# bcsefercik/markerless-robot-camera-calibration

Measured on AMD Instinct MI355X. Metric: point-cloud frames/sec at 200k pts/frame, higher is better.
Workload: dtype f32

## Files before the change

### markerless-robot-camera-calibration_amd/_lib.py

```python
import ctypes
import os
from ctypes import c_char_p, c_double, c_float, c_int, c_int64, c_size_t, c_void_p

import torch

_HERE = os.path.dirname(os.path.abspath(__file__))
ABI_VERSION = 4
LIB_PATH = os.environ.get("SVHIP_LIB") or os.path.join(_HERE, "libsvhip.so")

SV_ACT_NONE, SV_ACT_RELU, SV_ACT_LEAKY_RELU = 0, 1, 2
SV_POOL_MAX, SV_POOL_AVG = 0, 1
SV_REDUCE_MEAN, SV_REDUCE_FIRST = 0, 1
SV_TILE_ROWS = 128
SV_ERR_UNSUPPORTED = -5
SV_PN_MAX_LAYERS = 4
SV_PN_MAX_SCALES = 4
SV_BQ_MAX_RADII = 4
SV_GROUP_SSG, SV_GROUP_MSG = 0, 1
SV_LOSS_POSE, SV_LOSS_SHAPE_MATCH, SV_LOSS_POSE_MATCH, SV_LOSS_KP_POSE_MATCH = 0, 1, 2, 3
SV_AUG_STRIDE, SV_AUG_ELASTIC0, SV_AUG_ELASTIC1 = 40, 0, 7
SV_AUG_E_ON, SV_AUG_E_OFFSET, SV_AUG_E_BX, SV_AUG_E_BY, SV_AUG_E_BZ, SV_AUG_E_GRAN, SV_AUG_E_MAG = range(7)
SV_AUG_NOISE_ON, SV_AUG_NOISE_SIGMA, SV_AUG_NOISE_CLIP, SV_AUG_TRANSFORM_ON, SV_AUG_ROT, SV_AUG_TRANSLATION = 14, 15, 16, 17, 18, 27
SV_AUG_FLIP_SIGN, SV_AUG_GRAVITY_ON, SV_AUG_GRAVITY_ANGLE, SV_AUG_GRAVITY_COS, SV_AUG_GRAVITY_SIN = 30, 31, 32, 33, 34
SV_ORIGIN_NONE, SV_ORIGIN_CENTER, SV_ORIGIN_BASE = 0, 1, 2
SV_COORD_BIAS = 1 << 17
SV_COORD_BITS = 18
SV_MAX_BATCH = 1024
SV_FRAME_MAX_LEVELS, SV_FRAME_MAX_CUTS, SV_FRAME_RECORD = 8, 4, 16
SV_FRAME_K3, SV_FRAME_DOWN, SV_FRAME_UP, SV_FRAME_SPLIT = 1, 2, 4, 8
SV_FIELD_F32, SV_FIELD_F64 = 7, 8
SV_UNPACK_BIGENDIAN, SV_UNPACK_KEEP_NONFINITE = 1, 2
SV_DEPTH_U16, SV_DEPTH_F32 = 4, 7
SV_RGBD_ALIGNED, SV_RGBD_NEAREST, SV_RGBD_BGR = 1, 2, 4
SV_FRAME_REC_HASH, SV_FRAME_REC_K3, SV_FRAME_REC_DOWN, SV_FRAME_REC_UP, SV_FRAME_REC_SPLIT = 1, 2, 3, 4, 5


class SvHipError(RuntimeError):
    pass


_P = c_void_p
SIGNATURES = {
    "sv_last_error": (c_char_p, []),
    "sv_abi_version": (c_int, []),
    "sv_voxelize_workspace_bytes": (c_size_t, [c_int64]),
    "sv_voxelize": (c_int, [_P, c_int, c_int64, _P, c_size_t, _P, _P, _P, _P, _P, _P, _P]),
    "sv_voxel_reduce": (c_int, [_P, c_int, _P, _P, c_int64, c_int, _P, _P]),
    "sv_hash_build": (c_int, [_P, c_int64, _P, _P, c_int64, _P]),
    "sv_stride_map_workspace_bytes": (c_size_t, [c_int64]),
    "sv_stride_map": (c_int, [_P, c_int64, c_int, _P, c_size_t, _P, _P, _P, _P, _P, _P]),
    "sv_kernel_map_k3": (c_int, [_P, c_int64, c_int, c_int, _P, _P, c_int64, _P, c_int64, _P, _P]),
    "sv_kernel_map_down": (c_int, [_P, _P, c_int64, c_int, c_int64, _P, c_int64, _P, _P]),
    "sv_kernel_map_up": (c_int, [_P, _P, c_int64, c_int, _P, c_int64, _P, _P]),
    "sv_plan_workspace_bytes": (c_size_t, [c_int64]),
# ... 110 lines not shown
_lib = None


def load():
    global _lib
    if _lib is not None:
        return _lib
    if not os.path.exists(LIB_PATH):
        raise SvHipError(
            f"{LIB_PATH} not found: build it with `python -c 'import __graft_entry__ as g; g.build()'` "
            "(or `make -C markerless-robot-camera-calibration_amd/csrc`). There is no CPU fallback."
        )
    lib = ctypes.CDLL(LIB_PATH)
    lib.sv_abi_version.restype = c_int
    if lib.sv_abi_version() != ABI_VERSION:
        raise SvHipError(f"{LIB_PATH} has C-ABI version {lib.sv_abi_version()}, this package binds version {ABI_VERSION}: "
                         "rebuild it (`python -c 'import __graft_entry__ as g; g.build()'`)")
    for name, (res, args) in SIGNATURES.items():
        fn = getattr(lib, name)
        fn.restype = res
        fn.argtypes = args
    _lib = lib
    return lib


def _check(rc, name):
    if rc != 0:
        msg = _lib.sv_last_error().decode("utf-8", "replace")
        raise SvHipError(f"{name} failed with status {rc}: {msg}")


def ptr(t):
    if t is None:
        return None
    return c_void_p(t.data_ptr())


def stream_ptr():
    return c_void_p(torch.cuda.current_stream().cuda_stream)


def call(name, *args):
    lib = load()
    rc = getattr(lib, name)(*args)
    _check(rc, name)


def conv_last_instance():
    raw = load().sv_conv_last_instance().decode()
    name, _, flags = raw.partition("|")
    return name, {k: int(v) for k, v in (kv.split("=") for kv in flags.split(",") if kv)}


class conv_dispatch:

    def __init__(self, want_scale, tail_fraction=-1.0):
        self.args = (c_double(want_scale), c_double(tail_fraction))

    def __enter__(self):
        call("sv_conv_set_dispatch", *self.args)

    def __exit__(self, *exc):
        call("sv_conv_set_dispatch", c_double(-1.0), c_double(-1.0))


def require_cuda(t, what="tensor"):
    if not t.is_cuda:
        raise SvHipError(f"{what} must live on the GPU (got {t.device}); the HIP path has no CPU fallback")
    return t
```

### markerless-robot-camera-calibration_amd/csrc/sv_conv.hip

```cpp
#include <stdarg.h>
#include <stdio.h>
#include <stdlib.h>
#include <vector>

#include "sv_conv_params.h"

namespace sv {

static thread_local char g_last_instance[128] = "";
static thread_local double g_want_scale_override = -1.0;
static thread_local double g_tail_override = -1.0;
void note_instance(const char* fmt, ...) {
  va_list ap;
  va_start(ap, fmt);
  vsnprintf(g_last_instance, sizeof(g_last_instance), fmt, ap);
  va_end(ap);
}
#ifndef SV_CONV_WANT_SCALE_DEFAULT
#define SV_CONV_WANT_SCALE_DEFAULT 0.3
#endif
#ifndef SV_CONV_TAIL_DEFAULT
#define SV_CONV_TAIL_DEFAULT 0.15
#endif
constexpr int chunk_for(int tm, int waves_n) {
// ... 752 lines not shown
  SV_CHECK_ARG(in_ld >= Cin && out_ld >= Cout, "row strides too small");
  SV_CHECK_ARG(act >= SV_ACT_NONE && act <= SV_ACT_LEAKY_RELU, "bad activation");
  if (V_out == 0) return SV_OK;
  SV_CHECK_ARG(in && W && out, "null pointer");
  SV_CHECK_ARG(V_in >= 1, "V_in = rows of `in` (every index of the plan is below it)");
  const bool has_plan = perm || nbr_s || submask;
  SV_CHECK_ARG(!has_plan || (perm && nbr_s && submask), "perm, nbr_s and submask must be given together");
  SV_CHECK_ARG(has_plan || K == 1, "K > 1 needs a plan");
  SV_CHECK_ARG(!residual || res_ld >= Cout, "residual stride too small");
  ConvParams p;
  p.in = in; p.in_ld = in_ld; p.Cin = Cin; p.W = W; p.K = K; p.Cout = Cout;
  p.perm = perm; p.nbr_s = nbr_s; p.submask = submask; p.tile_order = tile_order; p.V_out = V_out; p.Vpad = Vpad;
  p.scale = scale; p.shift = shift; p.residual = residual; p.res_ld = res_ld;
  p.acc_init = acc_init; p.acc_ld = acc_ld;
  p.act = act; p.slope = slope; p.out = out; p.out_ld = out_ld;
  p.vec_a = (in_ld % 4 == 0) && (Cin % 4 == 0) && (((uintptr_t)in & 15) == 0);
  const uint64_t in_bytes = ((uint64_t)(V_in - 1) * (uint64_t)in_ld + (uint64_t)Cin) * 4u;
  const uint64_t w_bytes = (uint64_t)K * (uint64_t)Cin * (uint64_t)Cout * 4u;
  const uint64_t out_bytes = ((uint64_t)(V_out - 1) * (uint64_t)out_ld + (uint64_t)Cout) * 4u;
  const uint64_t res_bytes = residual ? ((uint64_t)(V_out - 1) * (uint64_t)res_ld + (uint64_t)Cout) * 4u : 0u;
  const uint64_t acc_bytes = acc_init ? ((uint64_t)(V_out - 1) * (uint64_t)acc_ld + (uint64_t)Cout) * 4u : 0u;
  p.buf_ok = in_bytes < BUF_LIMIT && w_bytes < BUF_LIMIT && out_bytes < BUF_LIMIT && res_bytes < BUF_LIMIT &&
             acc_bytes < BUF_LIMIT && (((uintptr_t)perm & 15) == 0);
  p.acc_bytes = p.buf_ok ? (uint32_t)acc_bytes : 0u;
  if (!p.buf_ok && !has_plan && K == 1 && w_bytes < BUF_LIMIT) {
    int64_t ld_max = in_ld > out_ld ? in_ld : out_ld;
    if (residual && res_ld > ld_max) ld_max = res_ld;
    const int64_t rows = (int64_t)((BUF_LIMIT - 4096u) / ((uint64_t)ld_max * 4u)) / PLAN_TILE * PLAN_TILE;
    if (rows >= PLAN_TILE && rows < V_out) {
      for (int64_t r0 = 0; r0 < V_out; r0 += rows) {
        const int64_t n = V_out - r0 < rows ? V_out - r0 : rows;
        const int rc = sv_conv_fwd_acc(in + r0 * in_ld, n, in_ld, Cin, W, K, Cout, nullptr, nullptr, nullptr, nullptr, n,
                                       (n + PLAN_TILE - 1) / PLAN_TILE * PLAN_TILE, acc_init ? acc_init + r0 * acc_ld : nullptr,
                                       acc_ld, scale, shift, residual ? residual + r0 * res_ld : nullptr, res_ld, act, slope,
                                       out + r0 * out_ld, out_ld, stream_);
        if (rc != SV_OK) return rc;
      }
      return SV_OK;
    }
  }
  p.in_bytes = p.buf_ok ? (uint32_t)in_bytes : 0u;
  p.w_bytes = p.buf_ok ? (uint32_t)w_bytes : 0u;
  p.out_bytes = p.buf_ok ? (uint32_t)out_bytes : 0u;
  p.res_bytes = p.buf_ok ? (uint32_t)res_bytes : 0u;
  p.ntiles = 0;
  p.ny = 0;
  p.trace = nullptr;
  p.main_blocks = 0;
  p.main_tiles128 = 0;
  if (has_plan && K > 1 && K <= 27 && Cin == 3 && Cout == 32 && !acc_init) {
    if (p.buf_ok) return launch_conv_first_mfma(p, stream);
    return launch_conv_first_layer(p, stream);
  }
  if (has_plan && K > 1 && K <= 32 && Cin == 32 && Cout == 32 && p.vec_a && p.buf_ok && !acc_init)
    return launch_conv_thin(p, stream, sv::g_want_scale_override >= 1.0);
  if (!has_plan && K == 1 && Cout <= 4 && p.vec_a && Cin >= 64 && !acc_init) return launch_linear_narrow(p, stream);
  return select_and_launch(p, stream);
}
```

### markerless-robot-camera-calibration_amd/csrc/sv_conv_params.h

```cpp
#pragma once
#include <type_traits>

#include "sv_common.h"

namespace sv {

typedef float f32x4 __attribute__((ext_vector_type(4)));

struct ConvParams {
  const float* in;
  int64_t in_ld;
  int Cin;
  const float* W;
  int K;
  int Cout;
  const int32_t* perm;
  const int32_t* nbr_s;
  const uint32_t* submask;
  const int32_t* tile_order;
  int64_t V_out;
  int64_t Vpad;
  const float* scale;
  const float* shift;
  const float* residual;
  int64_t res_ld;
  const float* acc_init;
  int64_t acc_ld;
  uint32_t acc_bytes;
  int act;
  float slope;
  float* out;
  int64_t out_ld;
  int vec_a;
  uint32_t in_bytes, w_bytes, out_bytes, res_bytes;
  int buf_ok;
  int ntiles;
  int ny;
  unsigned long long* trace;
  int main_blocks;
  int main_tiles128;
};

constexpr int PLAN_TILE = SV_TILE_ROWS;
void note_instance(const char* fmt, ...);
int launch_conv_first_mfma(const ConvParams& p, hipStream_t stream);
int launch_conv_first_layer(const ConvParams& p, hipStream_t stream);
int launch_conv_thin(const ConvParams& p, hipStream_t stream, bool alone);
int launch_linear_narrow(const ConvParams& p, hipStream_t stream);

constexpr uint32_t BUF_ABSENT = 0x80000000u;
constexpr uint32_t BUF_LIMIT = 0x7fff0000u;
typedef int i32x4_t __attribute__((ext_vector_type(4)));
typedef int i32x3_t __attribute__((ext_vector_type(3)));
typedef int i32x2_t __attribute__((ext_vector_type(2)));
template <int N>
__device__ __forceinline__ auto buffer_load_floats(__amdgpu_buffer_rsrc_t rsrc, uint32_t voffset, uint32_t soffset) {
  typedef float vec_t __attribute__((ext_vector_type(N)));
  if constexpr (N == 1) {
    vec_t r;
    r[0] = __builtin_bit_cast(float, __builtin_amdgcn_raw_buffer_load_b32(rsrc, voffset, soffset, 0));
    return r;
  } else if constexpr (N == 2) {
    return __builtin_bit_cast(vec_t, __builtin_amdgcn_raw_buffer_load_b64(rsrc, voffset, soffset, 0));
  } else if constexpr (N == 3) {
    return __builtin_bit_cast(vec_t, __builtin_amdgcn_raw_buffer_load_b96(rsrc, voffset, soffset, 0));
  } else {
    static_assert(N == 4, "1..4 floats per load");
    return __builtin_bit_cast(vec_t, __builtin_amdgcn_raw_buffer_load_b128(rsrc, voffset, soffset, 0));
  }
}

template <int MR>
__device__ __forceinline__ void load_perm_rows(const ConvParams& p, const int64_t rows0, const int lq, int (&o)[MR][4]) {
#pragma unroll
  for (int s = 0; s < MR; ++s) {
    const int64_t r = rows0 + s * 16 + lq * 4;
    if (p.perm) {
      const int4 o4 = *(const int4*)(p.perm + r);
      o[s][0] = o4.x;
      o[s][1] = o4.y;
      o[s][2] = o4.z;
      o[s][3] = o4.w;
    } else {
#pragma unroll
      for (int reg = 0; reg < 4; ++reg) o[s][reg] = (r + reg < p.V_out) ? (int)(r + reg) : -1;
    }
  }
}

template <int MR, int NT, bool PRELOADED = false>
__device__ __forceinline__ void epilogue_buffered(const ConvParams& p, const f32x4 (&acc)[MR][NT], const int64_t rows0,
                                                  const int lq, const int col0, const int (*o_pre)[4] = nullptr) {
  typedef float yvec_t __attribute__((ext_vector_type(NT)));
  const __amdgpu_buffer_rsrc_t rsrc_out = __builtin_amdgcn_make_buffer_rsrc((void*)p.out, 0, (int)p.out_bytes, 0x00020000);
  const __amdgpu_buffer_rsrc_t rsrc_res =
      __builtin_amdgcn_make_buffer_rsrc((void*)p.residual, 0, p.residual ? (int)p.res_bytes : 0, 0x00020000);
  int o[MR][4];
// ... 66 lines not shown
```

### markerless-robot-camera-calibration_amd/csrc/sv_conv_special.hip

```cpp
#include <stdio.h>
#include <stdlib.h>
#include <algorithm>
#include <vector>

#include "sv_conv_params.h"

namespace sv {

constexpr int NARROW_ROWS = 64;
template <int C>
__global__ __launch_bounds__(256) void linear_narrow_kernel(ConvParams p) {
  constexpr int ROWS = NARROW_ROWS, COLS = 32, SW = COLS + 1, LPT = ROWS / 32;
  __shared__ float tile[2][ROWS * SW];
  const int tid = threadIdx.x;
  const int64_t row0 = (int64_t)blockIdx.x * ROWS;
  const int Cin = p.Cin;
  const int lr = tid >> 3, lc = (tid & 7) * 4;
  float4 ra[LPT];
  auto load = [&](int c0) {
#pragma unroll
    for (int i = 0; i < LPT; ++i) {
      const int64_t r = row0 + lr + 32 * i;
      const int c = c0 + lc;
      const bool ok = r < p.V_out && c < Cin;
      const float4 v = *(const float4*)(p.in + (ok ? r * p.in_ld + c : 0));
      ra[i] = ok ? v : make_float4(0.f, 0.f, 0.f, 0.f);
    }
  };
  auto store = [&](float* dst) {
#pragma unroll
    for (int i = 0; i < LPT; ++i) {
      float* d = dst + (lr + 32 * i) * SW + lc;
      d[0] = ra[i].x;
      d[1] = ra[i].y;
      d[2] = ra[i].z;
      d[3] = ra[i].w;
    }
  };
  float acc[C];
#pragma unroll
  for (int j = 0; j < C; ++j) acc[j] = 0.0f;
  load(0);
  store(tile[0]);
  __syncthreads();
  int buf = 0;
  for (int c0 = 0; c0 < Cin; c0 += COLS) {
    const bool more = c0 + COLS < Cin;
    if (more) load(c0 + COLS);
    if (tid < ROWS) {
      const float* x = tile[buf] + tid * SW;
      const float* w = p.W + (int64_t)c0 * p.Cout;
      const int nc = min(COLS, Cin - c0);
#pragma unroll 8
      for (int c = 0; c < nc; ++c) {
// ... 359 lines not shown
    SV_HIP(hipGetDeviceProperties(&prop, dev));
    n_cu = prop.multiProcessorCount > 0 ? prop.multiProcessorCount : 256;
    SV_HIP(hipFuncSetAttribute((const void*)conv_thin_lds_kernel<32, 32, D, WAVES>, hipFuncAttributeMaxDynamicSharedMemorySize,
                               (int)(((size_t)27 * 32 * 32 + (size_t)WAVES * (32 * 16)) * sizeof(float))));
    attr_set = true;
  }
  const int n_sub = (int)(p.Vpad / 16);
  const int grid = n_sub < n_cu ? n_sub : n_cu;
  static const bool trace = getenv("SV_THIN_TRACE") != nullptr;
  ConvParams q = p;
  q.trace = nullptr;
  if (trace) {
    SV_HIP(hipMalloc((void**)&q.trace, (size_t)grid * WAVES * 12 * sizeof(unsigned long long)));
    SV_HIP(hipMemsetAsync(q.trace, 0, (size_t)grid * WAVES * 12 * sizeof(unsigned long long), stream));
  }
  hipLaunchKernelGGL((conv_thin_lds_kernel<32, 32, D, WAVES>), dim3((unsigned)grid), dim3(WAVES * 64), lds, stream, q, n_sub);
  note_instance("conv_thin_lds_kernel<32, 32>|fast=1,ring=0,full=1");
  SV_LAUNCH_CHECK();
  if (trace) {
    std::vector<unsigned long long> h((size_t)grid * WAVES * 12);
    SV_HIP(hipStreamSynchronize(stream));
    SV_HIP(hipMemcpy(h.data(), q.trace, h.size() * sizeof(unsigned long long), hipMemcpyDeviceToHost));
    SV_HIP(hipFree(q.trace));
    std::vector<double> stage, table, loop, store, life, per_off, it01, it12, pre;
    for (size_t w = 0; w < (size_t)grid * WAVES; ++w) {
      const unsigned long long* o = &h[w * 12];
      if (!o[0]) continue;
      if (o[8] && o[9] && o[10]) {
        pre.push_back((double)(o[8] - o[2]));
        it01.push_back((double)(o[9] - o[8]));
        it12.push_back((double)(o[10] - o[9]));
      }
      stage.push_back((double)(o[1] - o[0]));
      life.push_back((double)(o[5] - o[0]));
      if (o[6]) {
        table.push_back((double)(o[2] - o[1]));
        loop.push_back((double)(o[3] - o[2]));
        store.push_back((double)(o[4] - o[3]));
        if (o[7]) per_off.push_back((double)(o[3] - o[2]) / (double)o[7]);
      }
    }
    auto med = [](std::vector<double>& v) {
      if (v.empty()) return 0.0;
      std::sort(v.begin(), v.end());
      return v[v.size() / 2];
    };
    fprintf(stderr, "[thin trace] K=%d n_sub=%d grid=%d | median cycles: weights staged %.0f, first tile: table %.0f, loop %.0f "
            "(%.0f per offset; table staged -> loop %.0f, first 4 offsets %.0f, next 4 %.0f), store %.0f, wave life %.0f\n", p.K, n_sub,
            grid, med(stage), med(table), med(loop), med(per_off), med(pre), med(it01), med(it12), med(store), med(life));
  }
  return SV_OK;
}

int launch_conv_thin(const ConvParams& p, hipStream_t stream, bool alone) {
  if (alone && p.K <= 27 && (((uintptr_t)p.W) & 15) == 0) return launch_conv_thin_lds(p, stream);
  hipLaunchKernelGGL((conv_thin_kernel<32, 32, 1, 4>), dim3((unsigned)(p.Vpad / 64)), dim3(256), 0, stream, p);
  note_instance("conv_thin_kernel<32, 32>|fast=1,ring=0,full=1");
  SV_LAUNCH_CHECK();
  return SV_OK;
}

template <int CIN, int COUT, int SPLIT>
__global__ __launch_bounds__(256) void conv_first_layer_kernel(ConvParams p) {
  constexpr int CT = COUT / SPLIT;
  constexpr int KMAX = 27;
  const int tid = threadIdx.x;
  const int K = p.K;
  const int j0 = (int)blockIdx.y * CT;
  const float* __restrict__ w_s = p.W + j0;
  const int64_t r = (int64_t)blockIdx.x * 256 + tid;
  const bool in_range = r < p.Vpad;
  const int64_t o = in_range ? (int64_t)p.perm[r] : -1;
  float acc[CT];
#pragma unroll
  for (int j = 0; j < CT; ++j) acc[j] = 0.0f;
  int n[KMAX];
#pragma unroll
  for (int k = 0; k < KMAX; ++k) n[k] = (o >= 0 && k < K) ? p.nbr_s[(int64_t)k * p.Vpad + r] : -1;
  constexpr int G = 9;
#pragma unroll
  for (int k0 = 0; k0 < KMAX; k0 += G) {
    float x[G][CIN];
#pragma unroll
    for (int g = 0; g < G; ++g) {
      const float* src = p.in + (n[k0 + g] >= 0 ? (int64_t)n[k0 + g] * p.in_ld : 0);
#pragma unroll
      for (int c = 0; c < CIN; ++c) x[g][c] = src[c];
    }
#pragma unroll
    for (int g = 0; g < G; ++g) {
      const bool has = n[k0 + g] >= 0;
      if (__ballot(has) == 0ull) continue;
      const float* w = w_s + (k0 + g) * CIN * COUT;
      if (has) {
#pragma unroll
        for (int c = 0; c < CIN; ++c) {
#pragma unroll
          for (int j = 0; j < CT; ++j) acc[j] = __builtin_fmaf(x[g][c], w[c * COUT + j], acc[j]);
        }
      }
    }
  }
  if (o < 0) return;
  float* dst = p.out + o * p.out_ld + j0;
#pragma unroll
  for (int j = 0; j < CT; ++j) {
    float v = acc[j];
    if (p.scale)
// ... 51 lines not shown
```

### markerless-robot-camera-calibration_amd/nn.py

```python
import math
from ctypes import c_float, c_int, c_int64, c_size_t

import numpy as np
import torch
import torch.nn as nn

from . import _lib, profiling
from ._lib import SV_ACT_LEAKY_RELU, SV_ACT_NONE, SV_ACT_RELU, call, ptr, stream_ptr
from .sparse import SparseTensor, SplitPlan

KERNEL_OFFSET_PERMUTATION = None

import os as _os


def _parse_split_rules(text):
    rules = []
    for part in text.split(";"):
        if part.strip():
            rows, _, cuts = part.partition(":")
            cuts = tuple(int(v) for v in cuts.split(",") if v)
            rules.append((int(rows), cuts[0] if len(cuts) == 1 else cuts))
    return sorted(rules, key=lambda r: -r[0])


SPLIT_RULES = _parse_split_rules(_os.environ.get("MRCC_SPLIT_RULES", "20000:9,18"))
SPLIT_MIN_CHANNELS = int(_os.environ.get("MRCC_SPLIT_MIN_CHANNELS", "128"))


SPLIT_RULES_ONE_FRAME = _parse_split_rules(_os.environ.get("MRCC_SPLIT_RULES_ONE_FRAME", "50000:9,18"))


def split_points_for(rows):
    for min_rows, cuts in SPLIT_RULES:
        if rows >= min_rows:
            return cuts
    return None


def conv_forward(feats, weight3, plan, V_out, scale=None, shift=None, residual=None, act=SV_ACT_NONE, slope=0.01,
                 out=None, weight_bf16=None):
    K, Cin, Cout = weight3.shape
    if feats.shape[1] != Cin:
        raise ValueError(f"input has {feats.shape[1]} channels, kernel expects {Cin}")
    if feats.stride(1) != 1:
        feats = feats.contiguous()
    if out is None:
        out = torch.empty((V_out, Cout), dtype=torch.float32, device=feats.device)
    if isinstance(plan, SplitPlan):
        return _conv_forward_split(feats, weight3, plan, V_out, scale, shift, residual, act, slope, out, weight_bf16)
    return _conv_forward_one(feats, weight3, plan, V_out, scale, shift, residual, act, slope, out, None, wp=weight_bf16)


def pack_weights_bf16(weight3):
    K, Cin, Cout = weight3.shape
    w = weight3.detach().float().contiguous()
    wp = torch.empty(K * Cin * Cout, dtype=torch.bfloat16, device=w.device)
    call("sv_pack_weights_bf16", ptr(w), c_int(K), c_int(Cin), c_int(Cout), ptr(wp), stream_ptr())
    return wp


def _conv_forward_split(feats, weight3, plan, V_out, scale, shift, residual, act, slope, out, weight_bf16=None):
    K, Cin, Cout = weight3.shape
    timer = profiling.TIMER
    t0 = None
    if timer is not None:
        kname = profiling.conv_kernel_config(Cout, plan.Vpad, Cin, plan.parts[-1][1] - plan.parts[-1][0])
        if timer.want(kname):
            t0 = timer.start()
    if weight_bf16 is None and not weight3.is_contiguous():
        weight3 = weight3.contiguous()
    acc = None
    for i, (k0, k1, sub) in enumerate(plan.parts):
        w = weight3[k0:k1]
        wp = weight_bf16[k0 * Cin * Cout:k1 * Cin * Cout] if weight_bf16 is not None else None
        if i == len(plan.parts) - 1:
            _conv_forward_one(feats, w, sub, V_out, scale, shift, residual, act, slope, out, acc, timed=False, wp=wp)
        else:
            nxt = torch.empty((V_out, Cout), dtype=torch.float32, device=feats.device)
            _conv_forward_one(feats, w, sub, V_out, None, None, None, SV_ACT_NONE, slope, nxt, acc, timed=False, wp=wp)
            acc = nxt
    if t0 is not None:
# ... 284 lines not shown
            self._wpt = pack_weights_bf16((w.flip(0) if mirror else w).transpose(1, 2).contiguous())
            self._wpt_ver = ver
        return self._wpt


class _ConvBase(_Bf16Weights, nn.Module):
    def __init__(self, in_channels, out_channels, kernel_size=-1, stride=1, dilation=1, bias=False, dimension=3,
                 transposed=False):
        super().__init__()
        if dimension != 3:
            raise NotImplementedError("only dimension=3 (the reference passes D=3 everywhere)")
        self.in_channels, self.out_channels = in_channels, out_channels
        self.kernel_size, self.stride, self.dilation = kernel_size, stride, dilation
        self.dimension = dimension
        self.transposed = transposed
        self.kernel_volume = kernel_size ** dimension
        if self.kernel_volume > 1:
            self.kernel = nn.Parameter(torch.empty(self.kernel_volume, in_channels, out_channels))
        else:
            self.kernel = nn.Parameter(torch.empty(in_channels, out_channels))
        self.bias = nn.Parameter(torch.empty(1, out_channels)) if bias else None
        self.compute_precision = "fp32"
        self.training_precision = "fp32"
        self.reset_parameters()

    def reset_parameters(self):
        with torch.no_grad():
            n = (self.out_channels if self.transposed else self.in_channels) * self.kernel_volume
            stdv = 1.0 / math.sqrt(n)
            self.kernel.uniform_(-stdv, stdv)
            if self.bias is not None:
                self.bias.uniform_(-stdv, stdv)

    def weight3(self):
        w = self.kernel
        return w if w.dim() == 3 else w.unsqueeze(0)

    def packed_weights_bf16(self):
        return self._packed_bf16(self.kernel, self.weight3())

    def _load_from_state_dict(self, state_dict, prefix, local_metadata, strict, missing_keys, unexpected_keys,
                              error_msgs):
        key = prefix + "kernel"
        perm_table = KERNEL_OFFSET_PERMUTATION
        if perm_table is not None and key in state_dict and state_dict[key].dim() == 3:
            perm = perm_table.get(state_dict[key].shape[0]) if isinstance(perm_table, dict) else perm_table
            if perm is not None and len(perm) == state_dict[key].shape[0]:
                if sorted(perm) != list(range(len(perm))):
                    raise ValueError(f"KERNEL_OFFSET_PERMUTATION for kernel volume {len(perm)} is not a permutation")
                state_dict[key] = state_dict[key][torch.as_tensor(list(perm), device=state_dict[key].device)]
        super()._load_from_state_dict(state_dict, prefix, local_metadata, strict, missing_keys, unexpected_keys,
                                      error_msgs)

    def _plan(self, x):
        cm, ts = x.coordinate_manager, x.tensor_stride
        ks, st = self.kernel_size, self.stride
        if not self.transposed:
            if ks == 1 and st == 1:
                return None, ts
            if ks == 3 and st == 1:
                if self.dilation == 1 and self.in_channels >= SPLIT_MIN_CHANNELS and self.out_channels >= SPLIT_MIN_CHANNELS:
                    cuts = cm.split_cuts_for(cm.stride_map(ts).V)
                    if cuts is not None:
                        if cm.split_ready is not None:
                            torch.cuda.current_stream().wait_event(cm.split_ready)
                            cm.split_ready = None
                        return cm.plan_k3_split(ts, cuts), ts
                return cm.plan_k3(ts, self.dilation), ts
            if ks == 2 and st == 2:
                return cm.plan_down(ts), ts * 2
        else:
            if ks == 2 and st == 2:
                return cm.plan_up(ts), ts // 2
        raise NotImplementedError(
            f"kernel_size={ks} stride={st} transposed={self.transposed}: not used by the reference's U-Nets")

    def _grad_plan(self, x, plan):
        cm, ts = x.coordinate_manager, x.tensor_stride
        if self.kernel_size == 2 and self.stride == 2:
            return lambda: cm.plan_down(ts // 2) if self.transposed else cm.plan_up(ts * 2)
        return lambda: plan

    def forward_train(self, x, bn=None, residual=None, act=SV_ACT_NONE, slope=0.01, cat_with=None):
        plan, out_stride = self._plan(x)
        V_out = x.coordinate_manager.stride_map(out_stride).V
        mirror = self.kernel_size == 3
        out = sparse_conv(x.F, self.weight3(), self.bias, plan, V_out, self._grad_plan(x, plan), mirror, layer=self)
        if bn is not None:
            out = bn.bn(out)
        if residual is not None:
            out = out + (residual.F if isinstance(residual, SparseTensor) else residual)
        out = _act_torch(out, act, slope)
        if cat_with is not None:
            if cat_with.coordinate_manager is not x.coordinate_manager or cat_with.tensor_stride != out_stride:
                raise ValueError("ME.cat needs tensors on the same coordinate map")
            out = torch.cat([out, cat_with.F], dim=1)
        return x.new(out, tensor_stride=out_stride)

    def forward_fused(self, x, bn=None, residual=None, act=SV_ACT_NONE, slope=0.01, cat_with=None):
        if self.training or (bn is not None and bn.training):
            return self.forward_train(x, bn, residual, act, slope, cat_with)
        plan, out_stride = self._plan(x)
        V_out = x.coordinate_manager.stride_map(out_stride).V
        scale = shift = None
        if bn is not None:
            scale, shift = bn.folded()
            if self.bias is not None:
                raise NotImplementedError("conv bias followed by a fused BatchNorm")
        elif self.bias is not None:
            shift = self.bias.detach().reshape(-1)
        res = residual.F if isinstance(residual, SparseTensor) else residual
        wp = self._weight_bf16()
        bf16 = {} if wp is None else {"weight_bf16": wp}
        if cat_with is None:
            out = conv_forward(x.F, self.weight3().detach(), plan, V_out, scale, shift, res, act, slope, **bf16)
            return x.new(out, tensor_stride=out_stride)
        if cat_with.coordinate_manager is not x.coordinate_manager or cat_with.tensor_stride != out_stride:
            raise ValueError("ME.cat needs tensors on the same coordinate map")
        skip = cat_with.F
        C = self.out_channels
        buf = torch.empty((V_out, C + skip.shape[1]), dtype=torch.float32, device=x.F.device)
        conv_forward(x.F, self.weight3().detach(), plan, V_out, scale, shift, res, act, slope, out=buf[:, :C], **bf16)
        buf[:, C:].copy_(skip)
        return x.new(buf, tensor_stride=out_stride)

    def forward(self, x):
        return self.forward_fused(x)

    def extra_repr(self):
        return (f"in={self.in_channels}, out={self.out_channels}, kernel_size={self.kernel_size}, "
                f"stride={self.stride}, dilation={self.dilation}")


class MinkowskiConvolution(_ConvBase):
    def __init__(self, in_channels, out_channels, kernel_size=-1, stride=1, dilation=1, bias=False,
                 kernel_generator=None, expand_coordinates=False, convolution_mode=None, dimension=None):
        if dimension is None:
            raise ValueError("dimension is required")
        super().__init__(in_channels, out_channels, kernel_size, stride, dilation, bias, dimension, transposed=False)


class MinkowskiConvolutionTranspose(_ConvBase):
    def __init__(self, in_channels, out_channels, kernel_size=-1, stride=1, dilation=1, bias=False,
                 kernel_generator=None, expand_coordinates=False, convolution_mode=None, dimension=None):
        if dimension is None:
            raise ValueError("dimension is required")
        if expand_coordinates:
            raise NotImplementedError("expand_coordinates=True (generative transposed conv) is not on the hot path")
        super().__init__(in_channels, out_channels, kernel_size, stride, dilation, bias, dimension, transposed=True)


class MinkowskiBatchNorm(nn.Module):
    def __init__(self, num_features, eps=1e-5, momentum=0.1, affine=True, track_running_stats=True):
        super().__init__()
        self.bn = nn.BatchNorm1d(num_features, eps=eps, momentum=momentum, affine=affine,
# ... 176 lines not shown
```

### markerless-robot-camera-calibration_amd/sparse.py

```python
import threading
import weakref
from ctypes import c_float, c_int, c_int32, c_int64, c_size_t, c_void_p
from enum import Enum

import torch

from . import _lib
from ._lib import SV_TILE_ROWS, call, ptr, stream_ptr


class SparseTensorQuantizationMode(Enum):
    RANDOM_SUBSAMPLE = 0
    UNWEIGHTED_AVERAGE = 1
    UNWEIGHTED_SUM = 2
    NO_QUANTIZATION = 3


class MinkowskiAlgorithm(Enum):
    DEFAULT = 0
    MEMORY_EFFICIENT = 1
    SPEED_OPTIMIZED = 2


def _round_up(x, m):
# ... 149 lines not shown
        self.maps[stride] = m
        self.parents[stride // 2] = (parent[:V_in], child_start[: V + 1])
        return m

    def batch_bounds(self, stride):
        if stride not in self._batch_bounds:
            B = self.num_batches
            if B is None:
                m1 = self.stride_map(1)
                B = int(m1.coords[:, 0].max().item()) + 1 if m1.V else 1
                self.num_batches = B
            self._batch_bounds[stride] = self.batch_offsets(stride, B).tolist()
        return self._batch_bounds[stride]

    def _build_plan(self, nbr, ld, mask, K, V_out, nbr_base=0):
        dev = self.device
        Vpad = _round_up(max(V_out, 1), SV_TILE_ROWS)
        ws_bytes = _lib.load().sv_plan_workspace_bytes(c_int64(V_out))
        ws = torch.empty(ws_bytes, dtype=torch.uint8, device=dev)
        perm = torch.empty(Vpad, dtype=torch.int32, device=dev)
        nbr_s = torch.empty((K, Vpad), dtype=torch.int32, device=dev)
        submask = torch.empty((Vpad // SV_TILE_ROWS, K), dtype=torch.int32, device=dev)
        tile_order = torch.empty(Vpad // SV_TILE_ROWS, dtype=torch.int32, device=dev)
        call("sv_plan_build", ptr(nbr), c_int64(ld), ptr(mask), c_int(K), c_int64(V_out), c_int64(nbr_base), ptr(ws),
             c_size_t(ws_bytes),
             ptr(perm), ptr(nbr_s), ptr(submask), ptr(tile_order), c_int64(Vpad), stream_ptr())
        return ConvPlan(perm, nbr_s, submask, tile_order, V_out, Vpad, K)

    def plan_k3(self, stride, dilation=1):
        key = ("k3", stride, dilation)
        if key not in self.plans:
            m = self.stride_map(stride)
            tkeys, tvals, cap = m.hash()
            V = m.V
            nbr = torch.empty((27, max(V, 1)), dtype=torch.int32, device=self.device)
            mask = torch.empty(max(V, 1), dtype=torch.int32, device=self.device)
            call("sv_kernel_map_k3", ptr(m.coords), c_int64(V), c_int(stride), c_int(dilation), ptr(tkeys), ptr(tvals),
                 c_int64(cap), ptr(nbr), c_int64(max(V, 1)), ptr(mask), stream_ptr())
            self.plans[key] = self._own(self._build_plan(nbr, max(V, 1), mask, 27, V), nbr, max(V, 1), mask, stride, stride)
        return self.plans[key]

    def plan_k3_split(self, stride, split=14):
        cuts = (split,) if isinstance(split, int) else tuple(split)
        key = ("k3split", stride, split)
        if key not in self.plans:
            whole = self.plan_k3(stride)
            nbr, ld, mask = whole.raw
            parts = []
            bounds = (0,) + cuts + (27,)
            for k0, k1 in zip(bounds[:-1], bounds[1:]):
                sub = ((mask >> k0) & ((1 << (k1 - k0)) - 1)).to(torch.int32)
                plan = self._build_plan(nbr[k0:k1], ld, sub, k1 - k0, whole.V_out)
                parts.append((k0, k1, self._own(plan, nbr[k0:k1], ld, sub, stride, stride)))
            self.plans[key] = SplitPlan(parts, whole)
        return self.plans[key]

    def plan_down(self, stride):
        key = ("down", stride)
        if key not in self.plans:
            fine = self.stride_map(stride)
            coarse = self.stride_map(stride * 2)
            parent, _ = self.parents[stride]
            level = stride.bit_length() - 1
            Vc = coarse.V
            nbr = torch.empty((8, max(Vc, 1)), dtype=torch.int32, device=self.device)
            mask = torch.empty(max(Vc, 1), dtype=torch.int32, device=self.device)
            call("sv_kernel_map_down", ptr(fine.keys), ptr(parent), c_int64(fine.V), c_int(level), c_int64(Vc),
                 ptr(nbr), c_int64(max(Vc, 1)), ptr(mask), stream_ptr())
            self.plans[key] = self._own(self._build_plan(nbr, max(Vc, 1), mask, 8, Vc), nbr, max(Vc, 1), mask, stride,
                                        stride * 2)
        return self.plans[key]

    def plan_up(self, stride):
        key = ("up", stride)
        if key not in self.plans:
            fs = stride // 2
            if fs not in self.maps or fs not in self.parents:
                raise _lib.SvHipError(
                    f"transposed conv to tensor stride {fs}: that coordinate map does not exist "
                    "(ME semantics: the output reuses the encoder's map, model/backbone/minkunet.py:152-156)")
            fine = self.maps[fs]
            parent, _ = self.parents[fs]
            level = fs.bit_length() - 1
            V = fine.V
            nbr = torch.empty((8, max(V, 1)), dtype=torch.int32, device=self.device)
            mask = torch.empty(max(V, 1), dtype=torch.int32, device=self.device)
            call("sv_kernel_map_up", ptr(fine.keys), ptr(parent), c_int64(V), c_int(level), ptr(nbr),
                 c_int64(max(V, 1)), ptr(mask), stream_ptr())
            self.plans[key] = self._own(self._build_plan(nbr, max(V, 1), mask, 8, V), nbr, max(V, 1), mask, stride, fs)
        return self.plans[key]

    def split_cuts_for(self, rows):
        if self.split_rules is None:
            from . import nn as svnn

            return svnn.split_points_for(rows)
        for min_rows, cuts in self.split_rules:
            if rows >= min_rows:
                return cuts
        return None

    def build_plans(self, levels, k3=True, down=True, up=True, split=True):
        lib = _lib.load()
        L = levels
        ms = [self.stride_map(1 << l) for l in range(L + 1)]
        V = (c_int64 * (L + 1))(*[m.V for m in ms])
# ... 341 lines not shown
```

Measured before the change: 74.96.

## Split thin 32x32 k3 convs into 9-offset range passes with LDS-resident weights

Adds a conv_thin_range kernel that handles up to 9 kernel offsets per pass. It stages their weights in LDS, software-pipelines the gathers against MFMA, and can accumulate onto a previous pass's output through acc_init. In fused inference, 32->32 channel 3x3x3 convolutions now use a three-range split plan (0-9, 9-18, 18-27) built from slices of the shared neighbor map. The goal is to keep weights on-chip and raise occupancy compared with the single-pass thin kernels. The cost is extra output read-modify-write traffic and additional kernel launches per layer.

```diff
diff --git a/markerless-robot-camera-calibration_amd/_lib.py b/markerless-robot-camera-calibration_amd/_lib.py
--- a/markerless-robot-camera-calibration_amd/_lib.py
+++ b/markerless-robot-camera-calibration_amd/_lib.py
@@ -1,5 +1,6 @@
 import ctypes
 import os
+import threading
 from ctypes import c_char_p, c_double, c_float, c_int, c_int64, c_size_t, c_void_p
 
 import torch
@@ -216,6 +217,13 @@
     return name, {k: int(v) for k, v in (kv.split("=") for kv in flags.split(",") if kv)}
 
 
+_dispatch = threading.local()
+
+
+def dispatch_alone():
+    return getattr(_dispatch, "want_scale", -1.0) >= 1.0
+
+
 class conv_dispatch:
 
     def __init__(self, want_scale, tail_fraction=-1.0):
@@ -223,9 +231,11 @@
 
     def __enter__(self):
         call("sv_conv_set_dispatch", *self.args)
+        _dispatch.want_scale = self.args[0].value
 
     def __exit__(self, *exc):
         call("sv_conv_set_dispatch", c_double(-1.0), c_double(-1.0))
+        _dispatch.want_scale = -1.0
 
 
 def require_cuda(t, what="tensor"):
diff --git a/markerless-robot-camera-calibration_amd/csrc/sv_conv.hip b/markerless-robot-camera-calibration_amd/csrc/sv_conv.hip
--- a/markerless-robot-camera-calibration_amd/csrc/sv_conv.hip
+++ b/markerless-robot-camera-calibration_amd/csrc/sv_conv.hip
@@ -828,8 +828,10 @@
     if (p.buf_ok) return launch_conv_first_mfma(p, stream);
     return launch_conv_first_layer(p, stream);
   }
-  if (has_plan && K > 1 && K <= 32 && Cin == 32 && Cout == 32 && p.vec_a && p.buf_ok && !acc_init)
-    return launch_conv_thin(p, stream, sv::g_want_scale_override >= 1.0);
+  if (has_plan && K > 1 && K <= 32 && Cin == 32 && Cout == 32 && p.vec_a && p.buf_ok) {
+    const int rc = launch_conv_thin(p, stream, sv::g_want_scale_override >= 1.0);
+    if (rc != THIN_DECLINED) return rc;
+  }
   if (!has_plan && K == 1 && Cout <= 4 && p.vec_a && Cin >= 64 && !acc_init) return launch_linear_narrow(p, stream);
   return select_and_launch(p, stream);
 }
diff --git a/markerless-robot-camera-calibration_amd/csrc/sv_conv_params.h b/markerless-robot-camera-calibration_amd/csrc/sv_conv_params.h
--- a/markerless-robot-camera-calibration_amd/csrc/sv_conv_params.h
+++ b/markerless-robot-camera-calibration_amd/csrc/sv_conv_params.h
@@ -43,6 +43,7 @@
 
 constexpr int PLAN_TILE = SV_TILE_ROWS;
 void note_instance(const char* fmt, ...);
+constexpr int THIN_DECLINED = 1;
 int launch_conv_first_mfma(const ConvParams& p, hipStream_t stream);
 int launch_conv_first_layer(const ConvParams& p, hipStream_t stream);
 int launch_conv_thin(const ConvParams& p, hipStream_t stream, bool alone);
diff --git a/markerless-robot-camera-calibration_amd/csrc/sv_conv_special.hip b/markerless-robot-camera-calibration_amd/csrc/sv_conv_special.hip
--- a/markerless-robot-camera-calibration_amd/csrc/sv_conv_special.hip
+++ b/markerless-robot-camera-calibration_amd/csrc/sv_conv_special.hip
@@ -1,5 +1,6 @@
 #include <stdio.h>
 #include <stdlib.h>
+#include <string.h>
 #include <algorithm>
 #include <vector>
 
@@ -465,8 +466,163 @@
   return SV_OK;
 }
 
+constexpr int THIN_RANGE_MAX = 9;
+template <int CIN, int COUT, int D>
+__global__ __launch_bounds__(256) __attribute__((amdgpu_waves_per_eu(5))) void conv_thin_range_kernel(ConvParams p, int n_sub) {
+  constexpr int NT = COUT / 16, KS = CIN / 4, G4 = CIN / 16;
+  constexpr int ST = (THIN_RANGE_MAX * 16 + 63) / 64;
+  constexpr int W4 = THIN_RANGE_MAX * CIN * COUT / 4 / 256;
+  static_assert(CIN % 32 == 0 && COUT % 16 == 0 && NT >= 1 && NT <= 4 && D >= 1, "shape");
+  static_assert(THIN_RANGE_MAX * CIN * COUT % (4 * 256) == 0 && ST == 3, "staging");
+  typedef float bvec_t __attribute__((ext_vector_type(NT)));
+  extern __shared__ __attribute__((aligned(16))) float w_s[];
+  const int K = p.K;
+  const int tid = threadIdx.x;
+  const int lane = tid & 63;
+  const int wid = __builtin_amdgcn_readfirstlane(tid >> 6);
+  const int li = lane & 15, lq = lane >> 4;
+  const __amdgpu_buffer_rsrc_t rsrc_in = __builtin_amdgcn_make_buffer_rsrc((void*)p.in, 0, (int)p.in_bytes, 0x00020000);
+  const __amdgpu_buffer_rsrc_t rsrc_w = __builtin_amdgcn_make_buffer_rsrc((void*)p.W, 0, (int)p.w_bytes, 0x00020000);
+  const __amdgpu_buffer_rsrc_t rsrc_acc =
+      __builtin_amdgcn_make_buffer_rsrc((void*)p.acc_init, 0, p.acc_init ? (int)p.acc_bytes : 0, 0x00020000);
+  struct Tile {
+    int t128, sub;
+    int perm[1][4];
+    uint32_t sm;
+    int n_st[ST];
+  };
+  auto fetch = [&](int t, Tile& T) {
+    T.t128 = __builtin_amdgcn_readfirstlane(p.tile_order ? p.tile_order[t >> 3] : (t >> 3));
+    T.sub = t & 7;
+    const int64_t row0 = (int64_t)T.t128 * PLAN_TILE + T.sub * 16;
+    load_perm_rows<1>(p, row0, lq, T.perm);
+    T.sm = lane < K ? p.submask[(int64_t)T.t128 * K + lane] : 0u;
+#pragma unroll
+    for (int it = 0; it < ST; ++it) {
+      const int e = lane + 64 * it;
+      T.n_st[it] = e < K * 16 ? p.nbr_s[(int64_t)(e >> 4) * p.Vpad + row0 + (e & 15)] : -1;
+    }
+  };
+  const int t_step = (int)gridDim.x * 4;
+  int t = (int)blockIdx.x * 4 + wid;
+  Tile cur;
+  if (t < n_sub) fetch(t, cur);
+  {
+    f32x4 wv[W4];
+#pragma unroll
+    for (int i = 0; i < W4; ++i) wv[i] = buffer_load_floats<4>(rsrc_w, (uint32_t)(tid + 256 * i) * 16u, 0u);
+#pragma unroll
+    for (int i = 0; i < W4; ++i)
+      if (tid + 256 * i < K * (CIN * COUT / 4)) *(f32x4*)(w_s + (tid + 256 * i) * 4) = wv[i];
+  }
+  __syncthreads();
+  const float* w_lane = w_s + lq * COUT + NT * li;
+  for (; t < n_sub; t += t_step) {
+    auto row_offset = [&](int n) { return (int)(n >= 0 ? (uint32_t)n * (uint32_t)(p.in_ld * 4) : BUF_ABSENT); };
+    const int tab0 = row_offset(cur.n_st[0]), tab1 = row_offset(cur.n_st[1]), tab2 = row_offset(cur.n_st[2]);
+    const uint32_t amask = (uint32_t)__ballot((cur.sm >> cur.sub) & 1u);
+    const int nact = __builtin_popcount(amask);
+    const int64_t row0 = (int64_t)cur.t128 * PLAN_TILE + cur.sub * 16;
+    int o_pre[1][4] = {{cur.perm[0][0], cur.perm[0][1], cur.perm[0][2], cur.perm[0][3]}};
+    f32x4 acc[1][NT];
+#pragma unroll
+    for (int reg = 0; reg < 4; ++reg) {
+      const bvec_t v = buffer_load_floats<NT>(
+          rsrc_acc, o_pre[0][reg] >= 0 ? (uint32_t)o_pre[0][reg] * (uint32_t)(p.acc_ld * 4) + (uint32_t)(NT * li) * 4u : BUF_ABSENT, 0u);
+#pragma unroll
+      for (int n = 0; n < NT; ++n) acc[0][n][reg] = v[n];
+    }
+    if (nact > 0) {
+      float4 g[D][G4];
+      bvec_t b[2][KS / 2];
+      uint32_t t_rest = amask, w_rest = amask;
+      const int k_last = 31 - __builtin_clz(amask);
+      auto lookup = [&]() -> uint32_t {
+        const bool any = t_rest != 0u;
+        const int k = any ? __builtin_ctz(t_rest) : 0;
+        t_rest &= t_rest - 1u;
+        const int m1 = -((k >> 2) & 1), m2 = -((k >> 3) & 1);
+        int src = (tab0 & ~m1) | (tab1 & m1);
+        src = (src & ~m2) | (tab2 & m2);
+        const int off = __builtin_amdgcn_ds_bpermute((((k & 3) << 4) + li) << 2, src);
+        return any ? (uint32_t)off : BUF_ABSENT;
+      };
+      auto issue = [&](uint32_t off, float4 (&dst)[G4]) {
+#pragma unroll
+        for (int jj = 0; jj < G4; ++jj) {
+          const f32x4 v = buffer_load_floats<4>(rsrc_in, off + 16u * (uint32_t)lq, 64u * (uint32_t)jj);
+          dst[jj] = make_float4(v[0], v[1], v[2], v[3]);
+        }
+      };
+      auto next_wk = [&]() -> int {
+        const int k = w_rest ? __builtin_ctz(w_rest) : k_last;
+        w_rest &= w_rest - 1u;
+        return k;
+      };
+      auto load_w = [&](int k, int h, bvec_t (&dst)[KS / 2]) {
+        const float* wk = w_lane + k * (CIN * COUT) + h * (KS / 2) * 4 * COUT;
+#pragma unroll
+        for (int ks = 0; ks < KS / 2; ++ks) dst[ks] = *(const bvec_t*)(wk + 4 * ks * COUT);
+      };
+      auto compute = [&](float4 (&a)[G4], int h, bvec_t (&w)[KS / 2]) {
+#pragma unroll
+        for (int jj = 0; jj < G4 / 2; ++jj) {
+          const float4 av = a[h * (G4 / 2) + jj];
+          float am[4] = {av.x, av.y, av.z, av.w};
+          transpose4x4_lanegroups(am[0], am[1], am[2], am[3]);
+#pragma unroll
+          for (int m = 0; m < 4; ++m)
+#pragma unroll
+            for (int n = 0; n < NT; ++n)
+              acc[0][n] = __builtin_amdgcn_mfma_f32_16x16x4f32(am[m], w[4 * jj + m][n], acc[0][n], 0, 0, 0);
+        }
+      };
+#pragma unroll
+      for (int d = 0; d < D; ++d) issue(lookup(), g[d]);
+      uint32_t off_next = lookup();
+      int k_cur = next_wk();
+      load_w(k_cur, 0, b[0]);
+      for (int j0 = 0; j0 < nact; j0 += D) {
+#pragma unroll
+        for (int u = 0; u < D; ++u) {
+          load_w(k_cur, 1, b[1]);
+          const uint32_t off = off_next;
+          off_next = lookup();
+          __builtin_amdgcn_sched_barrier(0);
+          compute(g[u], 0, b[0]);
+          k_cur = next_wk();
+          load_w(k_cur, 0, b[0]);
+          __builtin_amdgcn_sched_barrier(0);
+          compute(g[u], 1, b[1]);
+          issue(off, g[u]);
+        }
+      }
+    }
+    epilogue_buffered<1, NT, true>(p, acc, row0, lq, NT * li, o_pre);
+    if (t + t_step < n_sub) fetch(t + t_step, cur);
+  }
+}
+
+static int launch_conv_thin_range(const ConvParams& p, hipStream_t stream) {
+  constexpr int D = 2;
+  constexpr int cap = 2048;
+  const int n_sub = (int)(p.Vpad / 16);
+  const int groups = n_sub / 4;
+  const size_t lds = (size_t)p.K * 32 * 32 * sizeof(float);
+  hipLaunchKernelGGL((conv_thin_range_kernel<32, 32, D>), dim3((unsigned)(groups < cap ? groups : cap)), dim3(256), lds, stream, p, n_sub);
+  note_instance("conv_thin_range_kernel<32, 32>|fast=1,ring=0,full=1");
+  SV_LAUNCH_CHECK();
+  return SV_OK;
+}
+
 int launch_conv_thin(const ConvParams& p, hipStream_t stream, bool alone) {
-  if (alone && p.K <= 27 && (((uintptr_t)p.W) & 15) == 0) return launch_conv_thin_lds(p, stream);
+  const char* force = getenv("SV_THIN_VARIANT");
+  const bool w16 = (((uintptr_t)p.W) & 15) == 0;
+  const bool f_l1 = force && !strcmp(force, "l1"), f_lds = force && !strcmp(force, "lds"), f_range = force && !strcmp(force, "range");
+  const bool range_ok = p.K <= THIN_RANGE_MAX && w16;
+  if (range_ok && !f_l1 && !f_lds && (p.acc_init || !alone || f_range)) return launch_conv_thin_range(p, stream);
+  if (p.acc_init) return THIN_DECLINED;
+  if ((alone || f_lds) && !f_l1 && p.K <= 27 && w16) return launch_conv_thin_lds(p, stream);
   hipLaunchKernelGGL((conv_thin_kernel<32, 32, 1, 4>), dim3((unsigned)(p.Vpad / 64)), dim3(256), 0, stream, p);
   note_instance("conv_thin_kernel<32, 32>|fast=1,ring=0,full=1");
   SV_LAUNCH_CHECK();
diff --git a/markerless-robot-camera-calibration_amd/nn.py b/markerless-robot-camera-calibration_amd/nn.py
--- a/markerless-robot-camera-calibration_amd/nn.py
+++ b/markerless-robot-camera-calibration_amd/nn.py
@@ -28,6 +28,7 @@
 SPLIT_MIN_CHANNELS = int(_os.environ.get("MRCC_SPLIT_MIN_CHANNELS", "128"))
 
 
+THIN_RANGE_PASSES = _os.environ.get("MRCC_THIN_RANGE_PASSES", "1") == "1"
 SPLIT_RULES_ONE_FRAME = _parse_split_rules(_os.environ.get("MRCC_SPLIT_RULES_ONE_FRAME", "50000:9,18"))
 
 
@@ -418,7 +419,7 @@
         super()._load_from_state_dict(state_dict, prefix, local_metadata, strict, missing_keys, unexpected_keys,
                                       error_msgs)
 
-    def _plan(self, x):
+    def _plan(self, x, fused=False):
         cm, ts = x.coordinate_manager, x.tensor_stride
         ks, st = self.kernel_size, self.stride
         if not self.transposed:
@@ -432,6 +433,8 @@
                             torch.cuda.current_stream().wait_event(cm.split_ready)
                             cm.split_ready = None
                         return cm.plan_k3_split(ts, cuts), ts
+                if fused and THIN_RANGE_PASSES and self.dilation == 1 and self.in_channels == 32 and self.out_channels == 32 and not _lib.dispatch_alone():
+                    return cm.plan_k3_ranges(ts), ts
                 return cm.plan_k3(ts, self.dilation), ts
             if ks == 2 and st == 2:
                 return cm.plan_down(ts), ts * 2
@@ -466,7 +469,7 @@
     def forward_fused(self, x, bn=None, residual=None, act=SV_ACT_NONE, slope=0.01, cat_with=None):
         if self.training or (bn is not None and bn.training):
             return self.forward_train(x, bn, residual, act, slope, cat_with)
-        plan, out_stride = self._plan(x)
+        plan, out_stride = self._plan(x, fused=True)
         V_out = x.coordinate_manager.stride_map(out_stride).V
         scale = shift = None
         if bn is not None:
diff --git a/markerless-robot-camera-calibration_amd/sparse.py b/markerless-robot-camera-calibration_amd/sparse.py
--- a/markerless-robot-camera-calibration_amd/sparse.py
+++ b/markerless-robot-camera-calibration_amd/sparse.py
@@ -225,6 +225,24 @@
                 sub = ((mask >> k0) & ((1 << (k1 - k0)) - 1)).to(torch.int32)
                 plan = self._build_plan(nbr[k0:k1], ld, sub, k1 - k0, whole.V_out)
                 parts.append((k0, k1, self._own(plan, nbr[k0:k1], ld, sub, stride, stride)))
+            self.plans[key] = SplitPlan(parts, whole)
+        return self.plans[key]
+
+    def plan_k3_ranges(self, stride, cuts=(9, 18)):
+        key = ("k3", stride, ("ranges",) + tuple(cuts))
+        if key not in self.plans:
+            whole = self.plan_k3(stride)
+            bounds = (0,) + tuple(cuts) + (whole.K,)
+            width = bounds[1] - bounds[0]
+            if all(k1 - k0 == width for k0, k1 in zip(bounds[:-1], bounds[1:])):
+                subs = whole.submask.view(-1, len(bounds) - 1, width).transpose(0, 1).contiguous()
+            else:
+                subs = [whole.submask[:, k0:k1].contiguous() for k0, k1 in zip(bounds[:-1], bounds[1:])]
+            parts = []
+            for i, (k0, k1) in enumerate(zip(bounds[:-1], bounds[1:])):
+                part = ConvPlan(whole.perm, whole.nbr_s[k0:k1], subs[i], whole.tile_order, whole.V_out, whole.Vpad, k1 - k0)
+                part.in_stride = part.out_stride = stride
+                parts.append((k0, k1, part))
             self.plans[key] = SplitPlan(parts, whole)
         return self.plans[key]
 
```

New measurement: 75.05, median of 6. About the same (+0.1%).
